# dellytools/delly

Hardware: AMD Instinct MI355X
Metric: candidate split-read alignments/sec (DEL, 150bp reads, 1kb ref window) (higher is better)
Workload: dtype int32-exact (uint8 / int16 storage)

## Files before the change

### delly_amd/csrc/sparse_needle.hpp

```cpp
#pragma once
#include <type_traits>

#ifndef DH_SP_CALLS
#define DH_SP_FN __forceinline__
#else
#define DH_SP_FN __noinline__
#endif

#include "split_kernel.hpp"

namespace dh {

constexpr int SP_NEG = -30000;
constexpr int SP_INF = 0x3fffffff;
constexpr int SP_LEVELS_MAX = 512;
constexpr int SP_UNKNOWN = -(1 << 30);

struct SparseWs {
  int16_t* frF;
  int16_t* frR;
  int32_t* cF;
  int32_t* cR;
  int32_t* runsF;
  int32_t* runsR;
  int32_t* listF;
  int32_t* listR;
  int32_t ndp;
  int32_t smax;
  int32_t pred_cap;
  int32_t runs_cap;
};

struct SparseRes {
  int resolved;
  int found;
  int unsplit;
  int best, consLeft, refLeft, refRight;
  int nrunsF, nrunsR;
  int levels;
  int mmF, mmR;
  unsigned long long t[5];
  int runF, runR;
};

typedef const __attribute__((address_space(1))) uint32_t* sp_gu32;
__device__ __forceinline__ int sp_ld16(const int16_t* p) {
  const uintptr_t u = reinterpret_cast<uintptr_t>(p);
  const uint32_t v = __hip_atomic_load((sp_gu32)(u & ~(uintptr_t)3), __ATOMIC_RELAXED, __HIP_MEMORY_SCOPE_AGENT);
  return (int)(int16_t)((u & 2) ? (v >> 16) : (v & 0xffffu));
}
__device__ __forceinline__ int sp_ld32(const int32_t* p) {
  return (int)__hip_atomic_load((sp_gu32) reinterpret_cast<uintptr_t>(p), __ATOMIC_RELAXED, __HIP_MEMORY_SCOPE_AGENT);
}

__device__ __forceinline__ int sp_ld8(const uint8_t* p) {
  const uintptr_t u = reinterpret_cast<uintptr_t>(p);
  const uint32_t v = __hip_atomic_load((sp_gu32)(u & ~(uintptr_t)3), __ATOMIC_RELAXED, __HIP_MEMORY_SCOPE_AGENT);
  return (int)((v >> (8 * (u & 3))) & 0xffu);
}

struct FrGlobal16 {
  const int16_t* base;
  int ndp;
  __device__ __forceinline__ int get(int d, int q) const { return sp_ld16(base + (size_t)d * ndp + q); }
};
struct FrTile8 {
  const uint8_t* base;
  int ndp;
  const uint8_t* row0;
  const uint8_t* row1;
  int S;
  __device__ __forceinline__ int get(int d, int q) const {
    return (d >= S - 1) ? (int)((d & 1) ? row1 : row0)[q] - 1 : sp_ld8(base + (size_t)d * ndp + q) - 1;
  }
};

__device__ __forceinline__ uint64_t sp_load8(const uint8_t* p) {
  uint64_t v;
  __builtin_memcpy(&v, p, 8);
  return v;
}

__device__ __forceinline__ uint64_t sp_lds8u(const uint8_t* p) {
  uint64_t v;
  __builtin_memcpy(&v, p, 8);
  return v;
}

constexpr int SP_LB = 16;
template <int TW, int STRCAP, typename ELEM = int16_t, int NROWS = 3>
struct __attribute__((aligned(16))) SpTileT {
  typedef ELEM elem_t;
  static constexpr int tw = TW;
  static constexpr int row_len = TW + 2 * SP_LB + 64;
  static constexpr int str_cap = STRCAP;
  static constexpr bool narrow = sizeof(ELEM) == 1;
  ELEM row[2][NROWS][TW + 2 * SP_LB + 64];
  uint8_t str[STRCAP > 0 ? STRCAP : 8];
};
typedef SpTileT<960, 8192, int16_t, 2> SpTile;

template <typename TILE, bool STAGED>
__device__ __forceinline__ void sp_tile_levels(const uint8_t* aF, const uint8_t* bF, const uint8_t* aR, const uint8_t* bR, int c0, int m, int n,
                                               int d0, int nl, int tlo, int thi, int16_t* FRf, int16_t* FRr, int ndp, TILE& T,
                                               int16_t* reachF, int16_t* reachR, int lane) {
  constexpr int OFF = SP_LB + 1;
  const int ND = n + m + 1;
  const int base = tlo - OFF;
  auto ld8 = [&](const uint8_t* p) -> uint64_t { return STAGED ? sp_lds8a(p) : sp_load8(p); };
  for (int j = 0; j < nl; ++j) {
    const int d = d0 + j;
    const int halo = nl - 1 - j;
    const int qa = max(tlo - halo, 0), qb = min(thi + halo, ND);
    int16_t* curF = T.row[0][d & 1] - base;
    int16_t* curR = T.row[1][d & 1] - base;
    const int16_t* p1F = T.row[0][(d + 1) & 1] - base;
    const int16_t* p1R = T.row[1][(d + 1) & 1] - base;
    const int16_t* p2F = curF;
    const int16_t* p2R = curR;
    int16_t* gF = FRf + (size_t)d * ndp;
    int16_t* gR = FRr + (size_t)d * ndp;
    const int seed = (d == 0) ? 0 : -1;
    int rf = -1, rr = -1;
    for (int q0 = qa; q0 < qb; q0 += 2 * WAVE) {
      int bf[2], br[2], kk[2];
      uint64_t zf[2], zr[2];
#pragma unroll
      for (int u = 0; u < 2; ++u) {
        const int q = min(q0 + u * WAVE + lane, qb - 1);
        const int k = q - m;
        kk[u] = k;
        const int nk = n - k, rmax = min(m, nk);
        const int first = (k < 0 && -2 * k <= d) ? -k : ((k >= 0) ? seed : -1);
        bf[u] = br[u] = first;
        if (d > 0) {
          {
            const int v1 = p1F[q], v1l = p1F[q - 1], v2 = p2F[q], v2r = p2F[q + 1];
            int b = max(v1, first);
            if ((unsigned)v1l <= (unsigned)nk) b = max(b, v1l);
            if (v2 >= 0) b = max(b, min(v2 + 1, rmax));
            if (v2r >= 0 && v2r < m) b = max(b, v2r + 1);
            bf[u] = b;
          }
          {
            const int v1 = p1R[q], v1l = p1R[q - 1], v2 = p2R[q], v2r = p2R[q + 1];
            int b = max(v1, first);
            if ((unsigned)v1l <= (unsigned)nk) b = max(b, v1l);
            if (v2 >= 0) b = max(b, min(v2 + 1, rmax));
            if (v2r >= 0 && v2r < m) b = max(b, v2r + 1);
            br[u] = b;
          }
        }
        const int r0 = max(bf[u], 0), r1 = max(br[u], 0);
        zf[u] = ld8(aF + r0) ^ ld8(bF + (max(r0 + k, c0) - c0));
        zr[u] = ld8(aR + r1) ^ ld8(bR + (max(r1 + k, c0) - c0));
      }
      int endF[2], endR[2];
      bool moreF[2], moreR[2];
#pragma unroll
      for (int u = 0; u < 2; ++u) {
        const int k = kk[u];
        {
          const int b0 = max(bf[u], 0);
          const int lim = min(m - b0, n - b0 - k);
          const int adv = zf[u] ? (int)(__builtin_ctzll(zf[u]) >> 3) : 8;
          endF[u] = b0 + lim;
          moreF[u] = bf[u] >= 0 && adv >= 8 && lim > 8;
          bf[u] = (bf[u] < 0) ? -1 : b0 + min(adv, lim);
        }
        {
          const int b0 = max(br[u], 0);
          const int lim = min(m - b0, n - b0 - k);
          const int adv = zr[u] ? (int)(__builtin_ctzll(zr[u]) >> 3) : 8;
          endR[u] = b0 + lim;
          moreR[u] = br[u] >= 0 && adv >= 8 && lim > 8;
          br[u] = (br[u] < 0) ? -1 : b0 + min(adv, lim);
        }
      }
#pragma unroll
      for (int u = 0; u < 2; ++u) {
        const int q = q0 + u * WAVE + lane, k = kk[u];
        if (__ballot(moreF[u])) {
          if (moreF[u]) {
            int r = bf[u];
            for (;;) {
              const uint64_t z = ld8(aF + r) ^ ld8(bF + (r + k - c0));
              if (z) { r += (int)(__builtin_ctzll(z) >> 3); break; }
              r += 8;
              if (r >= endF[u]) break;
            }
            bf[u] = min(r, endF[u]);
          }
        }
        if (__ballot(moreR[u])) {
          if (moreR[u]) {
            int r = br[u];
            for (;;) {
              const uint64_t z = ld8(aR + r) ^ ld8(bR + (r + k - c0));
              if (z) { r += (int)(__builtin_ctzll(z) >> 3); break; }
              r += 8;
              if (r >= endR[u]) break;
            }
            br[u] = min(r, endR[u]);
          }
        }
        if (q < qb) {
          curF[q] = (int16_t)bf[u];
          curR[q] = (int16_t)br[u];
          if (q >= tlo && q < thi) {
            gF[q] = (int16_t)bf[u];
            gR[q] = (int16_t)br[u];
            rf = max(rf, bf[u]);
            rr = max(rr, br[u]);
          }
        }
      }
    }
#pragma unroll
    for (int o = 32; o >= 1; o >>= 1) {
      rf = max(rf, __shfl_xor(rf, o));
      rr = max(rr, __shfl_xor(rr, o));
    }
    if (lane == 0) {
      reachF[d] = (int16_t)max((int)reachF[d], rf < 0 ? SP_NEG : rf);
      reachR[d] = (int16_t)max((int)reachR[d], rr < 0 ? SP_NEG : rr);
    }
// ... 47 lines not shown
}

#ifdef DH_SPS_DBG
__device__ unsigned long long dh_dbg[16];
#define DH_DBG_ADD(i, v) do { if (lane == 0) atomicAdd(&dh_dbg[i], (unsigned long long)(v)); } while (0)
#define DH_DBG_T() wall_clock64()
#else
#define DH_DBG_ADD(i, v) do { } while (0)
#define DH_DBG_T() 0ull
#endif
#ifdef DH_SPS_FINE
__shared__ unsigned long long dh_tl[6];
#define DH_TL(i) do { if (lane == 0) dh_tl[i] = wall_clock64(); } while (0)
#else
#define DH_TL(i) do { } while (0)
#endif
constexpr int SPS_OFF = 20;

template <bool NEG, bool EDGE>
__device__ __forceinline__ uint32_t sps_entries4(const uint8_t* cons, const uint8_t* ref, uint32_t e1, uint32_t e1l, uint32_t e2, uint32_t e2r,
                                                 int qb, int m, int n, int dhalf, int seed1, int ND, int& maxB, uint32_t& pend, int pbit) {
  int Bv[4], r0v[4], rmaxv[4];
  uint64_t zv[4];
#pragma unroll
  for (int i = 0; i < 4; ++i) {
    const int q = qb + i, k = q - m;
    const int E1 = (int)((e1 >> (8 * i)) & 255u), E1L = (int)((e1l >> (8 * i)) & 255u);
    const int E2 = (int)((e2 >> (8 * i)) & 255u), E2R = (int)((e2r >> (8 * i)) & 255u);
    int rmax = m;
    int B = E1;
    if (EDGE) {
      const int nk = n - k;
      rmax = min(m, nk);
      if ((unsigned)(E1L - 1) <= (unsigned)nk) B = max(B, E1L);
    } else {
      B = max(B, E1L);
    }
    B = max(B, E2 ? min(E2 + 1, rmax + 1) : 0);
    B = max(B, ((unsigned)(E2R - 1) < (unsigned)m) ? E2R + 1 : 0);
    if (NEG) {
      const int kk = -k;
      if ((unsigned)(kk - 1) < (unsigned)dhalf) B = max(B, kk + 1);
      B = max(B, (k >= 0) ? seed1 : 0);
    } else {
      B = max(B, seed1);
    }
    Bv[i] = B;
    rmaxv[i] = rmax;
    r0v[i] = max(B - 1, 0);
  }
#pragma unroll
  for (int i = 0; i < 4; ++i) {
    const int k = qb + i - m;
    zv[i] = sp_lds8a(cons + r0v[i]) ^ sp_lds8a(ref + (NEG ? max(r0v[i] + k, 0) : r0v[i] + k));
  }
  uint32_t outw = 0;
#pragma unroll
  for (int i = 0; i < 4; ++i) {
    const int q = qb + i;
    const int adv = zv[i] ? (int)(__builtin_ctzll(zv[i]) >> 3) : 8;
    int NB = Bv[i] ? min(r0v[i] + adv, rmaxv[i]) + 1 : 0;
    bool more = (Bv[i] != 0) && (adv >= 8) && (rmaxv[i] - r0v[i] > 8);
    if (EDGE) {
      NB = (q < ND) ? NB : 0;
      more = more && (q < ND);
    }
    outw |= (uint32_t)NB << (8 * i);
    maxB = max(maxB, NB);
    pend |= (more ? 1u : 0u) << (pbit + i);
  }
  return outw;
}

__device__ __forceinline__ void sps_extend_pending(const uint8_t* consF, const uint8_t* refF, const uint8_t* consR, const uint8_t* refR,
                                                   uint8_t* curF, uint8_t* curR, int q0, int m, int n, uint32_t pend, int& maxB_F,
                                                   int& maxB_R, int lane) {
  int total = 0;
#pragma unroll
  for (int e = 0; e < 8; ++e) total += __popcll(__ballot((pend >> e) & 1u));
  if (total > 6) {
#pragma unroll
    for (int e = 0; e < 8; ++e) {
      const bool mine = (pend >> e) & 1u;
      if (__ballot(mine) == 0ull) continue;
      if (mine) {
        const bool rev = e >= 4;
        const int q = q0 + 4 * lane + (e & 3), k = q - m;
        const uint8_t* cons = rev ? consR : consF;
        const uint8_t* ref = rev ? refR : refF;
        uint8_t* cur = rev ? curR : curF;
        const int end = min(m, n - k);
        int r = (int)cur[q] - 1;
        for (;;) {
          const uint64_t z = sp_lds8a(cons + r) ^ sp_lds8a(ref + r + k);
          if (z) { r += (int)(__builtin_ctzll(z) >> 3); break; }
          r += 8;
          if (r >= end) break;
        }
        r = min(r, end);
        cur[q] = (uint8_t)(r + 1);
        if (rev) maxB_R = max(maxB_R, r + 1); else maxB_F = max(maxB_F, r + 1);
      }
    }
    return;
  }
  unsigned long long lanes = __ballot(pend != 0u);
  while (lanes) {
    const int src = __builtin_ctzll(lanes);
    lanes &= lanes - 1;
    uint32_t bits = (uint32_t)__builtin_amdgcn_readlane((int)pend, src);
    while (bits) {
      const int e = __builtin_ctz(bits);
      bits &= bits - 1;
      const bool rev = e >= 4;
      const int q = q0 + 4 * src + (e & 3), k = q - m;
      const uint8_t* cons = rev ? consR : consF;
      const uint8_t* ref = rev ? refR : refF;
      uint8_t* cur = rev ? curR : curF;
      const int end = min(m, n - k);
      int r = (int)cur[q] - 1;
      for (;;) {
        const int rr = r + 8 * lane;
        uint64_t z = 0;
        if (rr < end) z = sp_lds8a(cons + rr) ^ sp_lds8a(ref + rr + k);
        const unsigned long long stop = __ballot(rr >= end || z != 0ull);
        if (stop == 0ull) { r += 8 * WAVE; continue; }
        const int jl = __builtin_ctzll(stop);
        const int rj = r + 8 * jl;
        const uint32_t zlo = (uint32_t)__builtin_amdgcn_readlane((int)(uint32_t)(z & 0xffffffffull), jl);
        const uint32_t zhi = (uint32_t)__builtin_amdgcn_readlane((int)(uint32_t)(z >> 32), jl);
        const uint64_t zz = ((uint64_t)zhi << 32) | zlo;
        r = (rj >= end) ? end : min(rj + (zz ? (int)(__builtin_ctzll(zz) >> 3) : 8), end);
        break;
      }
      if (lane == 0) cur[q] = (uint8_t)(r + 1);
      if (rev) maxB_R = max(maxB_R, r + 1); else maxB_F = max(maxB_F, r + 1);
    }
  }
}

template <bool NEG, bool EDGE, bool L0>
__device__ __forceinline__ uint32_t sps_level_step(const uint8_t* consF, const uint8_t* refF, const uint8_t* consR, const uint8_t* refR, int m, int n,
                                               int d, int q0, int ND, uint8_t* curF, uint8_t* curR, const uint8_t* p1F, const uint8_t* p1R,
                                               uint8_t* gF, uint8_t* gR, int& maxB_F, int& maxB_R, int lane) {
  const int qb = q0 + 4 * lane;
  uint32_t e1F = 0, e1lF = 0, e2F = 0, e2rF = 0, e1R = 0, e1lR = 0, e2R = 0, e2rR = 0;
  if (!L0) {
    const uint32_t* a1F = reinterpret_cast<const uint32_t*>(p1F + qb);
    const uint32_t* a2F = reinterpret_cast<const uint32_t*>(curF + qb);
    const uint32_t* a1R = reinterpret_cast<const uint32_t*>(p1R + qb);
    const uint32_t* a2R = reinterpret_cast<const uint32_t*>(curR + qb);
    e1F = a1F[0]; e1lF = __builtin_amdgcn_alignbyte(e1F, a1F[-1], 3u); e2F = a2F[0]; e2rF = __builtin_amdgcn_alignbyte(a2F[1], e2F, 1u);
    e1R = a1R[0]; e1lR = __builtin_amdgcn_alignbyte(e1R, a1R[-1], 3u); e2R = a2R[0]; e2rR = __builtin_amdgcn_alignbyte(a2R[1], e2R, 1u);
    if (d >= 2 && qb < ND) {
      *reinterpret_cast<uint32_t*>(gF + qb) = e2F;
      *reinterpret_cast<uint32_t*>(gR + qb) = e2R;
    }
  }
  uint32_t pend = 0;
  const int seed1 = L0 ? 1 : 0, dhalf = d >> 1;
  const uint32_t oF = sps_entries4<NEG, EDGE>(consF, refF, e1F, e1lF, e2F, e2rF, qb, m, n, dhalf, seed1, ND, maxB_F, pend, 0);
  __builtin_amdgcn_sched_barrier(0);
  const uint32_t oR = sps_entries4<NEG, EDGE>(consR, refR, e1R, e1lR, e2R, e2rR, qb, m, n, dhalf, seed1, ND, maxB_R, pend, 4);
  if (qb < ND) {
    *reinterpret_cast<uint32_t*>(curF + qb) = oF;
    *reinterpret_cast<uint32_t*>(curR + qb) = oR;
  }
  return pend;
}

template <typename TILE>
__device__ DH_SP_FN void sps_level_block(const uint8_t* consF, const uint8_t* refF, const uint8_t* consR, const uint8_t* refR, int m,
                                         int n, int d0, int d1, int16_t* FRf, int16_t* FRr, int ndp, TILE& T, int16_t* reachF,
                                         int16_t* reachR, int lane) {
  static_assert(TILE::narrow, "byte rows");
  static_assert(sizeof(T.row[0][0]) % 4 == 0 && SPS_OFF % 4 == 0, "dword access to the tile rows");
  const int ND = n + m + 1;
  const unsigned long long tz0 = DH_DBG_T();
  DH_TL(0);
  if (d0 == 0) {
    static_assert(sizeof(T.row) % 16 == 0 && alignof(TILE) >= 16, "the tile is cleared sixteen bytes per lane and store");
    uint4* z = reinterpret_cast<uint4*>(&T.row[0][0][0]);
    for (int i = lane; i < (int)(sizeof(T.row) / 16); i += WAVE) z[i] = make_uint4(0u, 0u, 0u, 0u);
  }
  __syncthreads();
  DH_TL(1);
  DH_DBG_ADD(0, 1);
  DH_DBG_ADD(7, DH_DBG_T() - tz0);
  for (int d = d0; d <= d1; ++d) {
    const unsigned long long tl0 = DH_DBG_T();
    uint8_t* curF = T.row[0][d & 1] + SPS_OFF;
    uint8_t* curR = T.row[1][d & 1] + SPS_OFF;
    const uint8_t* p1F = T.row[0][(d + 1) & 1] + SPS_OFF;
    const uint8_t* p1R = T.row[1][(d + 1) & 1] + SPS_OFF;
    uint8_t* gF = reinterpret_cast<uint8_t*>(FRf) + (size_t)max(d - 2, 0) * ndp;
    uint8_t* gR = reinterpret_cast<uint8_t*>(FRr) + (size_t)max(d - 2, 0) * ndp;
    int maxB_F = 0, maxB_R = 0;
    for (int q0 = 0; q0 < ND; q0 += 4 * WAVE) {
      const bool neg = q0 < m;
      const bool edge = q0 + 4 * WAVE - 1 > n;
      uint32_t pend;
      if (d == 0) {
        if (neg || edge) pend = sps_level_step<true, true, true>(consF, refF, consR, refR, m, n, d, q0, ND, curF, curR, p1F, p1R, gF, gR, maxB_F, maxB_R, lane);
        else pend = sps_level_step<false, false, true>(consF, refF, consR, refR, m, n, d, q0, ND, curF, curR, p1F, p1R, gF, gR, maxB_F, maxB_R, lane);
      } else if (neg || edge) {
        pend = sps_level_step<true, true, false>(consF, refF, consR, refR, m, n, d, q0, ND, curF, curR, p1F, p1R, gF, gR, maxB_F, maxB_R, lane);
      } else {
        pend = sps_level_step<false, false, false>(consF, refF, consR, refR, m, n, d, q0, ND, curF, curR, p1F, p1R, gF, gR, maxB_F, maxB_R, lane);
      }
      if (__ballot(pend != 0u)) {
        const unsigned long long te = DH_DBG_T();
        sps_extend_pending(consF, refF, consR, refR, curF, curR, q0, m, n, pend, maxB_F, maxB_R, lane);
        DH_DBG_ADD(5, 1);
        DH_DBG_ADD(6, DH_DBG_T() - te);
      }
    }
    const unsigned long long tl1 = DH_DBG_T();
    DH_TL(2);
#pragma unroll
    for (int o = 32; o >= 1; o >>= 1) {
      maxB_F = max(maxB_F, __shfl_xor(maxB_F, o));
      maxB_R = max(maxB_R, __shfl_xor(maxB_R, o));
    }
    if (lane == 0) {
      reachF[d] = (int16_t)(maxB_F <= 0 ? SP_NEG : maxB_F - 1);
      reachR[d] = (int16_t)(maxB_R <= 0 ? SP_NEG : maxB_R - 1);
    }
    __syncthreads();
    DH_DBG_ADD(1, 1);
    DH_DBG_ADD(2, tl1 - tl0);
    DH_DBG_ADD(3, DH_DBG_T() - tl1);
  }
  const unsigned long long tw0 = DH_DBG_T();
  if (d1 >= 2) asm volatile("s_waitcnt vmcnt(0)" ::: "memory");
  __syncthreads();
  DH_TL(3);
  DH_DBG_ADD(4, DH_DBG_T() - tw0);
}

template <typename TILE>
__device__ DH_SP_FN void sps_level_block_v1(const uint8_t* consF, const uint8_t* refF, const uint8_t* consR, const uint8_t* refR, int m,
                                             int n, int d0, int d1, int16_t* FRf, int16_t* FRr, int ndp, TILE& T, int16_t* reachF,
                                             int16_t* reachR, int lane) {
  static_assert(TILE::narrow, "byte rows");
  constexpr int OFF = SPS_OFF;
  const int ND = n + m + 1;
  if (d0 == 0) {
    uint32_t* z = reinterpret_cast<uint32_t*>(&T.row[0][0][0]);
    for (int i = lane; i < (int)(sizeof(T.row) / 4); i += WAVE) z[i] = 0u;
  }
  __syncthreads();
  for (int d = d0; d <= d1; ++d) {
    uint8_t* curF = T.row[0][d & 1] + OFF;
    uint8_t* curR = T.row[1][d & 1] + OFF;
    const uint8_t* p1F = T.row[0][(d + 1) & 1] + OFF;
    const uint8_t* p2F = curF;
    const uint8_t* p1R = T.row[1][(d + 1) & 1] + OFF;
    const uint8_t* p2R = curR;
    uint8_t* gF = reinterpret_cast<uint8_t*>(FRf) + (size_t)max(d - 2, 0) * ndp;
    uint8_t* gR = reinterpret_cast<uint8_t*>(FRr) + (size_t)max(d - 2, 0) * ndp;
    const int seed = (d == 0) ? 0 : -1;
    int rf = -1, rr = -1;
    for (int q0 = 0; q0 < ND; q0 += 2 * WAVE) {
      int bf[2], br[2], kk[2];
      uint64_t zf[2], zr[2];
#pragma unroll
      for (int u = 0; u < 2; ++u) {
        const int q = min(q0 + u * WAVE + lane, ND - 1);
        const int k = q - m;
        kk[u] = k;
        const int nk = n - k, rmax = min(m, nk);
        const int first = (k < 0 && -2 * k <= d) ? -k : ((k >= 0) ? seed : -1);
        bf[u] = br[u] = first;
        if (d > 0) {
          if (d >= 2 && q0 + u * WAVE + lane < ND) {
            gF[q] = p2F[q];
            gR[q] = p2R[q];
          }
          {
            const int e1 = p1F[q], e1l = p1F[q - 1], e2 = p2F[q], e2r = p2F[q + 1];
            int b = max(e1 - 1, first);
            if ((unsigned)(e1l - 1) <= (unsigned)nk) b = max(b, e1l - 1);
            if (e2 >= 1) b = max(b, min(e2, rmax));
            if (e2r >= 1 && e2r <= m) b = max(b, e2r);
            bf[u] = b;
          }
          {
            const int e1 = p1R[q], e1l = p1R[q - 1], e2 = p2R[q], e2r = p2R[q + 1];
            int b = max(e1 - 1, first);
            if ((unsigned)(e1l - 1) <= (unsigned)nk) b = max(b, e1l - 1);
            if (e2 >= 1) b = max(b, min(e2, rmax));
            if (e2r >= 1 && e2r <= m) b = max(b, e2r);
            br[u] = b;
          }
        }
        const int r0 = max(bf[u], 0), r1 = max(br[u], 0);
        zf[u] = sp_lds8u(consF + r0) ^ sp_lds8u(refF + max(r0 + k, 0));
        zr[u] = sp_lds8u(consR + r1) ^ sp_lds8u(refR + max(r1 + k, 0));
      }
      int endF[2], endR[2];
      bool moreF[2], moreR[2];
#pragma unroll
      for (int u = 0; u < 2; ++u) {
        const int k = kk[u];
        {
          const int b0 = max(bf[u], 0);
          const int lim = min(m - b0, n - b0 - k);
          const int adv = zf[u] ? (int)(__builtin_ctzll(zf[u]) >> 3) : 8;
          endF[u] = b0 + lim;
          moreF[u] = bf[u] >= 0 && adv >= 8 && lim > 8;
          bf[u] = (bf[u] < 0) ? -1 : b0 + min(adv, lim);
        }
        {
          const int b0 = max(br[u], 0);
          const int lim = min(m - b0, n - b0 - k);
          const int adv = zr[u] ? (int)(__builtin_ctzll(zr[u]) >> 3) : 8;
          endR[u] = b0 + lim;
          moreR[u] = br[u] >= 0 && adv >= 8 && lim > 8;
          br[u] = (br[u] < 0) ? -1 : b0 + min(adv, lim);
        }
      }
#pragma unroll
      for (int u = 0; u < 2; ++u) {
        const int q = q0 + u * WAVE + lane, k = kk[u];
        if (__ballot(moreF[u])) {
          if (moreF[u]) {
            int r = bf[u];
            for (;;) {
              const uint64_t z = sp_lds8u(consF + r) ^ sp_lds8u(refF + r + k);
              if (z) { r += (int)(__builtin_ctzll(z) >> 3); break; }
              r += 8;
              if (r >= endF[u]) break;
            }
            bf[u] = min(r, endF[u]);
          }
        }
        if (__ballot(moreR[u])) {
          if (moreR[u]) {
            int r = br[u];
            for (;;) {
              const uint64_t z = sp_lds8u(consR + r) ^ sp_lds8u(refR + r + k);
              if (z) { r += (int)(__builtin_ctzll(z) >> 3); break; }
              r += 8;
              if (r >= endR[u]) break;
            }
            br[u] = min(r, endR[u]);
          }
        }
        if (q < ND) {
          curF[q] = (uint8_t)(bf[u] + 1);
          curR[q] = (uint8_t)(br[u] + 1);
          rf = max(rf, bf[u]);
          rr = max(rr, br[u]);
        }
      }
    }
#pragma unroll
    for (int o = 32; o >= 1; o >>= 1) {
      rf = max(rf, __shfl_xor(rf, o));
      rr = max(rr, __shfl_xor(rr, o));
    }
    if (lane == 0) {
      reachF[d] = (int16_t)(rf < 0 ? SP_NEG : rf);
      reachR[d] = (int16_t)(rr < 0 ? SP_NEG : rr);
    }
    __syncthreads();
  }
  asm volatile("s_waitcnt vmcnt(0)" ::: "memory");
  __syncthreads();
}

__device__ __forceinline__ void sp_offer_chunk(int32_t* row, int rlo, int rhi, int k, int v, int& pm, int lane) {
  if (__ballot(v > pm && v >= rlo) == 0ull) return;
  int incl = v;
#pragma unroll
  for (int o = 1; o < WAVE; o <<= 1) {
    const int t = __shfl_up(incl, o);
    if (lane >= o) incl = max(incl, t);
  }
  int excl = __shfl_up(incl, 1);
  if (lane == 0) excl = SP_NEG;
  const int from = max(max(excl, pm) + 1, rlo), to = min(v, rhi);
  const int hs = min(to, from + 7);
  for (int r = from; r <= hs; ++r) atomicMin(&row[r], r + k);
  unsigned long long todo = __ballot(to > from + 7);
  while (todo) {
    const int src = __builtin_ctzll(todo);
    todo &= todo - 1;
    const int f2 = __shfl(from, src) + 8, t2 = __shfl(to, src), k2 = __shfl(k, src);
    for (int r = f2 + lane; r <= t2; r += WAVE) atomicMin(&row[r], r + k2);
  }
  pm = max(pm, __shfl(incl, WAVE - 1));
}
template <typename FRV>
__device__ __forceinline__ void sp_offer_negative(const FRV& FR, int32_t* row, int m, int d, int rlo, int rhi, int lane) {
  const int nneg = min(d / 2, m);
  for (int i0 = 0; i0 < nneg; i0 += WAVE) {
    const int i = i0 + lane;
    const int v = (i < nneg) ? FR.get(d, m - 1 - i) : SP_NEG;
    const int cnt = min(WAVE, nneg - i0);
    for (int t = 0; t < cnt; ++t) {
      const int vt = __shfl(v, t), kt = -(i0 + t + 1);
      const int lo = max(rlo, -kt), hi = min(vt, rhi);
      for (int r = lo + lane; r <= hi; r += WAVE) atomicMin(&row[r], r + kt);
    }
  }
}

template <typename FRV>
__device__ DH_SP_FN void sp_first_columns(const FRV& FR, int m, int n, int S, int rlo, int rhi, int32_t* cT, int lane) {
  const int ND = n + m + 1;
  const int rows = rhi - rlo + 1;
  for (int d = 0; d <= S; ++d)
    for (int i = lane; i < rows; i += WAVE) cT[(size_t)d * (m + 1) + rlo + i] = SP_INF;
  asm volatile("s_waitcnt vmcnt(0)" ::: "memory");
  __syncthreads();
  for (int d0 = 0; d0 <= S; d0 += 4) {
    int pm[4];
#pragma unroll
    for (int u = 0; u < 4; ++u) {
      pm[u] = (d0 + u <= S) ? rlo - 1 : rhi;
      if (d0 + u <= S) sp_offer_negative(FR, cT + (size_t)(d0 + u) * (m + 1), m, d0 + u, rlo, rhi, lane);
    }
    for (int q0 = m; q0 < ND && (pm[0] < rhi || pm[1] < rhi || pm[2] < rhi || pm[3] < rhi); q0 += WAVE) {
      const int q = q0 + lane;
      int v[4];
#pragma unroll
      for (int u = 0; u < 4; ++u) v[u] = (q < ND && pm[u] < rhi) ? FR.get(min(d0 + u, S), q) : SP_NEG;
#pragma unroll
      for (int u = 0; u < 4; ++u)
        if (pm[u] < rhi) sp_offer_chunk(cT + (size_t)(d0 + u) * (m + 1), rlo, rhi, q - m, v[u], pm[u], lane);
    }
  }
  asm volatile("s_waitcnt vmcnt(0)" ::: "memory");
  __syncthreads();
}

template <typename FRV>
__device__ DH_SP_FN int sp_deep_list(const FRV& FR, int m, int n, int S, int rlo, int32_t* list, int cap, int lane) {
  const int ND = n + m + 1;
  int cnt = 0;
  for (int q0 = 0; q0 < ND; q0 += WAVE) {
    const int q = q0 + lane;
    const bool hit = (q < ND) && (FR.get(S, min(q, ND - 1)) >= rlo);
    const unsigned long long bm = __ballot(hit);
    if (bm) {
      const unsigned long long below = (lane == 0) ? 0ull : (~0ull >> (64 - lane));
      const int pos = cnt + __popcll(bm & below);
      if (hit && pos < cap) list[pos] = q;
      cnt += __popcll(bm);
    }
  }
  asm volatile("s_waitcnt vmcnt(0)" ::: "memory");
  __syncthreads();
  return (cnt <= cap) ? cnt : -1;
}

template <bool WAIT = true>
__device__ __forceinline__ int sps_deep_list(const uint8_t* lv, int ND, int rlo, int32_t* list, int cap, int lane) {
  int cnt = 0;
  for (int q0 = 0; q0 < ND; q0 += WAVE) {
    const int q = q0 + lane;
    const bool hit = (q < ND) && ((int)lv[min(q, ND - 1)] - 1 >= rlo);
    const unsigned long long bm = __ballot(hit);
    if (bm) {
      const unsigned long long below = (lane == 0) ? 0ull : (~0ull >> (64 - lane));
      const int pos = cnt + __popcll(bm & below);
      if (hit && pos < cap) list[pos] = q;
      cnt += __popcll(bm);
    }
  }
  if (WAIT) {
    asm volatile("s_waitcnt vmcnt(0)" ::: "memory");
    __syncthreads();
  }
  return (cnt <= cap) ? cnt : -1;
}

template <typename FRV>
__device__ DH_SP_FN void sp_first_columns_list(const FRV& FR, int m, int S, int rlo, int rhi, const int32_t* list,
                                                   int cnt, int32_t* cT, int lane) {
  const int rows = rhi - rlo + 1;
  for (int d = 0; d <= S; ++d)
    for (int i = lane; i < rows; i += WAVE) cT[(size_t)d * (m + 1) + rlo + i] = SP_INF;
  asm volatile("s_waitcnt vmcnt(0)" ::: "memory");
  __syncthreads();
  if (cnt <= WAVE) {
    const int q = (lane < cnt) ? sp_ld32(list + lane) : -1;
    const bool use = q >= m;
    for (int d0 = 0; d0 <= S; d0 += 4) {
      int v[4];
#pragma unroll
      for (int u = 0; u < 4; ++u) v[u] = (use && d0 + u <= S) ? FR.get(d0 + u, q) : SP_NEG;
#pragma unroll
      for (int u = 0; u < 4; ++u) {
        if (d0 + u <= S) {
          int pm = rlo - 1;
          sp_offer_chunk(cT + (size_t)(d0 + u) * (m + 1), rlo, rhi, q - m, v[u], pm, lane);
        }
      }
    }
  } else {
    for (int d = 0; d <= S; ++d) {
      int pm = rlo - 1;
      for (int i0 = 0; i0 < cnt && pm < rhi; i0 += WAVE) {
        const int i = i0 + lane;
        const int q = (i < cnt) ? sp_ld32(list + i) : -1;
        const int v = (q >= m) ? FR.get(d, q) : SP_NEG;
        sp_offer_chunk(cT + (size_t)d * (m + 1), rlo, rhi, q - m, v, pm, lane);
      }
    }
  }
  for (int d = 2; d <= S; ++d) sp_offer_negative(FR, cT + (size_t)d * (m + 1), m, d, rlo, rhi, lane);
  asm volatile("s_waitcnt vmcnt(0)" ::: "memory");
  __syncthreads();
}

template <typename FRV>
__device__ DH_SP_FN void sp_first_columns_both(const FRV& FRf, const FRV& FRr, int m, int S, int rloF, int rhiF,
                                                   const int32_t* listF, int cntF, int32_t* cF, int rloR, int rhiR,
                                                   const int32_t* listR, int cntR, int32_t* cR, int lane) {
  const int rows = rhiF - rloF + 1;
  for (int d = 0; d <= S; ++d)
    for (int i = lane; i < rows; i += WAVE) {
      cF[(size_t)d * (m + 1) + rloF + i] = SP_INF;
      cR[(size_t)d * (m + 1) + rloR + i] = SP_INF;
    }
  asm volatile("s_waitcnt vmcnt(0)" ::: "memory");
  __syncthreads();
  const int qF = (lane < cntF) ? sp_ld32(listF + lane) : -1;
  const int qR = (lane < cntR) ? sp_ld32(listR + lane) : -1;
  const bool useF = qF >= m, useR = qR >= m;
  for (int d0 = 0; d0 <= S; d0 += 4) {
    int vF[4], vR[4];
#pragma unroll
    for (int u = 0; u < 4; ++u) {
      vF[u] = (useF && d0 + u <= S) ? FRf.get(d0 + u, qF) : SP_NEG;
      vR[u] = (useR && d0 + u <= S) ? FRr.get(d0 + u, qR) : SP_NEG;
    }
#pragma unroll
    for (int u = 0; u < 4; ++u) {
      if (d0 + u <= S) {
        int pmF = rloF - 1, pmR = rloR - 1;
        sp_offer_chunk(cF + (size_t)(d0 + u) * (m + 1), rloF, rhiF, qF - m, vF[u], pmF, lane);
        sp_offer_chunk(cR + (size_t)(d0 + u) * (m + 1), rloR, rhiR, qR - m, vR[u], pmR, lane);
      }
    }
  }
  for (int d = 2; d <= S; ++d) {
    sp_offer_negative(FRf, cF + (size_t)d * (m + 1), m, d, rloF, rhiF, lane);
    sp_offer_negative(FRr, cR + (size_t)d * (m + 1), m, d, rloR, rhiR, lane);
  }
  asm volatile("s_waitcnt vmcnt(0)" ::: "memory");
  __syncthreads();
}

template <typename FRV, bool REGRUNS = false>
__device__ DH_SP_FN int sp_trace(const FRV& FR, int m, int n, int r, int c, int D, int32_t* runs, int cap, int lane,
                                     int* mismatches = nullptr, int* runreg = nullptr) {
  const int ND = n + m + 1;
  const int D0 = rfl(D);
  int nv = 0, nh = 0;
  auto fr = [&](int d, int q) -> int { return (d < 0 || q < 0 || q >= ND) ? SP_NEG : FR.get(d, q); };
  int nruns = 0, last_op = -1, last_len = 0;
  auto emit = [&](int op, int len) {
    if (len <= 0) return;
    if (op == last_op) { last_len += len; return; }
    if (last_op >= 0) {
      if (REGRUNS) { if (lane == nruns) *runreg = (last_op << 24) | last_len; }
      else if (nruns < cap && lane == 0) runs[nruns] = (last_op << 24) | last_len;
      ++nruns;
    }
    last_op = op;
    last_len = len;
  };
  r = rfl(r); c = rfl(c); D = rfl(D);
  while (r > 0 || c > 0) {
    if (r == 0) { emit(2, c); c = 0; break; }
    if (c == 0) { emit(1, r); nv += r; r = 0; break; }
    const int k = c - r, q = k + m;
    if (D >= 2 && rfl(fr(D - 2, q + 1)) >= r - 1) { emit(1, 1); ++nv; --r; D -= 2; continue; }
    if (D >= 1 && rfl(fr(D - 1, q - 1)) >= r) { emit(2, 1); ++nh; --c; D -= 1; continue; }
    const int lowD = (D >= 1) ? max(rfl(fr(D - 1, q)) + 1, 0) : 0;
    int T = SP_NEG;
    if (D >= 2) T = max(T, rfl(fr(D - 2, q + 1)) + 1);
    if (D >= 1) T = max(T, rfl(fr(D - 1, q - 1)));
    const int start = max(0, -k);
    const int y = max(max(lowD, T + 1), start + 1);
    const int cnt = r - y + 1;
    emit(0, cnt);
    r -= cnt;
    c -= cnt;
    if (r < lowD) {
      int e = D - 1;
      while (e >= 1 && rfl(fr(e - 1, q)) >= r) --e;
      D = (rfl(fr(e, q)) >= r) ? e : D;
    }
  }
  if (last_op >= 0) {
    if (REGRUNS) { if (lane == nruns) *runreg = (last_op << 24) | last_len; }
    else if (nruns < cap && lane == 0) runs[nruns] = (last_op << 24) | last_len;
    ++nruns;
  }
  if (mismatches) *mismatches = (D0 - 2 * nv - nh) / 2;
  if (!REGRUNS) {
    asm volatile("s_waitcnt vmcnt(0)" ::: "memory");
    __syncthreads();
  }
  return (nruns <= (REGRUNS ? WAVE : cap)) ? nruns : -1;
}

struct SpsSmall {
  int qF, qR, nF, nR;
  uint32_t pF[3], pR[3];
};

template <typename FRV>
__device__ __forceinline__ bool sps_lists_small(const FRV& frF, const FRV& frR, const uint8_t* lvF, const uint8_t* lvR, int ND, int m, int SE,
                                                int rlo, int rloR, SpsSmall& Q, int lane) {
  Q.qF = Q.qR = -1;
  int nF = 0, nR = 0;
  for (int q0 = 0; q0 < ND; q0 += 4 * WAVE) {
    const int qb = q0 + 4 * lane;
    const uint32_t wf = *reinterpret_cast<const uint32_t*>(lvF + qb), wr = *reinterpret_cast<const uint32_t*>(lvR + qb);
    uint32_t hf = 0u, hr = 0u;
#pragma unroll
    for (int i = 0; i < 4; ++i) {
      const bool in = qb + i < ND;
      hf |= (uint32_t)(in && (int)((wf >> (8 * i)) & 255u) - 1 >= rlo) << i;
      hr |= (uint32_t)(in && (int)((wr >> (8 * i)) & 255u) - 1 >= rloR) << i;
    }
    if (__ballot((hf | hr) != 0u) == 0ull) continue;
#pragma unroll
    for (int i = 0; i < 4; ++i) {
      unsigned long long bf = __ballot((hf >> i) & 1u), br = __ballot((hr >> i) & 1u);
      if (nF + __popcll(bf) > WAVE || nR + __popcll(br) > WAVE) return false;
      while (bf) {
        const int b = __builtin_ctzll(bf);
        bf &= bf - 1;
        Q.qF = (lane == nF) ? q0 + 4 * b + i : Q.qF;
        ++nF;
      }
      while (br) {
        const int b = __builtin_ctzll(br);
        br &= br - 1;
        Q.qR = (lane == nR) ? q0 + 4 * b + i : Q.qR;
        ++nR;
      }
    }
  }
  Q.nF = nF;
  Q.nR = nR;
#pragma unroll
  for (int w = 0; w < 3; ++w) { Q.pF[w] = 0u; Q.pR[w] = 0u; }
#pragma unroll
  for (int d = 0; d < 9; ++d) {
    if (d <= SE) {
      const int vf = (Q.qF >= 0) ? frF.get(d, Q.qF) + 1 : 0;
      const int vr = (Q.qR >= 0) ? frR.get(d, Q.qR) + 1 : 0;
      Q.pF[d >> 2] |= (uint32_t)(vf & 255) << (8 * (d & 3));
      Q.pR[d >> 2] |= (uint32_t)(vr & 255) << (8 * (d & 3));
    }
  }
  return true;
}

template <int NL>
__device__ __forceinline__ void sps_row_best(const int (&lo_)[9], const int (&c2_)[9], int SE, int n, int r, long long& kb, int& db) {
  int thr[NL];
#pragma unroll
  for (int q = 0; q < NL; ++q) thr[q] = (q <= SE) ? ((c2_[q] > n) ? -1 : n - c2_[q]) : SP_INF;
#pragma unroll
  for (int d = 0; d < NL; ++d) {
    const int lo = lo_[d];
    int e = 0;
#pragma unroll
    for (int q = 0; q < NL; ++q) e += (int)(lo > thr[q]);
    const long long kk = ((long long)(d + e) << 40) | ((long long)r << 20) | (long long)lo;
    const bool take = (bool)((int)(d <= SE) & (int)(lo <= n) & (int)(e <= SE) & (int)(d + e <= SE) & (int)(kk <= kb));
    kb = take ? kk : kb;
    db = take ? d : db;
  }
}

template <int NL>
__device__ __forceinline__ void sps_join_small_t(const SpsSmall& Q, int m, int n, int SE, int rlo, int rhi, long long& key, int& dsel, int lane) {
  key = 0x7fffffffffffffffll;
  int dbest = 0;
  for (int r0 = rlo; r0 <= rhi; r0 += WAVE) {
    const int r = r0 + lane, rr = m - r;
    int lo_[9], c2_[9];
#pragma unroll
    for (int d = 0; d < 9; ++d) { lo_[d] = SP_INF; c2_[d] = SP_INF; }
    for (int t = 0; t < Q.nF; ++t) {
      const int k = __builtin_amdgcn_readlane(Q.qF, t) - m;
      const uint32_t p0 = (uint32_t)__builtin_amdgcn_readlane((int)Q.pF[0], t), p1 = (uint32_t)__builtin_amdgcn_readlane((int)Q.pF[1], t),
                     p2 = (uint32_t)__builtin_amdgcn_readlane((int)Q.pF[2], t);
      const bool on = r + k >= 0;
#pragma unroll
      for (int d = 0; d < NL; ++d) {
        if (d <= SE) {
          const int v = (int)((((d < 4) ? p0 : (d < 8) ? p1 : p2) >> (8 * (d & 3))) & 255u) - 1;
          lo_[d] = min(lo_[d], ((int)on & (int)(v >= r)) ? r + k : SP_INF);
        }
      }
    }
    for (int t = 0; t < Q.nR; ++t) {
      const int k = __builtin_amdgcn_readlane(Q.qR, t) - m;
      const uint32_t p0 = (uint32_t)__builtin_amdgcn_readlane((int)Q.pR[0], t), p1 = (uint32_t)__builtin_amdgcn_readlane((int)Q.pR[1], t),
                     p2 = (uint32_t)__builtin_amdgcn_readlane((int)Q.pR[2], t);
      const bool on = rr + k >= 0;
#pragma unroll
      for (int d = 0; d < NL; ++d) {
        if (d <= SE) {
          const int v = (int)((((d < 4) ? p0 : (d < 8) ? p1 : p2) >> (8 * (d & 3))) & 255u) - 1;
          c2_[d] = min(c2_[d], ((int)on & (int)(v >= rr)) ? rr + k : SP_INF);
        }
      }
    }
    if (r <= rhi) {
      long long kb = 0x7fffffffffffffffll;
      int db = 0;
      sps_row_best<NL>(lo_, c2_, SE, n, r, kb, db);
      if (kb < key) { key = kb; dbest = db; }
    }
  }
  long long kmin = key;
#pragma unroll
  for (int o = 32; o >= 1; o >>= 1) {
    const int lo = __shfl_xor((int)(kmin & 0xffffffffll), o), hi = __shfl_xor((int)(kmin >> 32), o);
    const long long w = ((long long)hi << 32) | (unsigned int)lo;
    kmin = w < kmin ? w : kmin;
  }
  const unsigned long long who = __ballot(key == kmin && key != 0x7fffffffffffffffll);
  dsel = who ? __shfl(dbest, __builtin_ctzll(who)) : 0;
  key = kmin;
}
__device__ __forceinline__ void sps_join_small(const SpsSmall& Q, int m, int n, int SE, int rlo, int rhi, long long& key, int& dsel, int lane) {
  if (SE <= 0) sps_join_small_t<1>(Q, m, n, SE, rlo, rhi, key, dsel, lane);
  else if (SE <= 2) sps_join_small_t<3>(Q, m, n, SE, rlo, rhi, key, dsel, lane);
  else sps_join_small_t<9>(Q, m, n, SE, rlo, rhi, key, dsel, lane);
}

template <typename TILE, bool LDSSTR>
__device__ DH_SP_FN SparseRes sparse_long_needle(const uint8_t* cons, const uint8_t* rcons, const uint8_t* ref, const uint8_t* rref,
                                                    int m, int n, const SparseWs& W, TILE& T, int16_t* reachF, int16_t* reachR,
                                                    int s_first, int lane) {
  SparseRes O;
  O.resolved = 0; O.found = 0; O.unsplit = SP_UNKNOWN; O.best = 0; O.consLeft = O.refLeft = O.refRight = 0; O.nrunsF = O.nrunsR = 0; O.levels = 0; O.mmF = O.mmR = 0;
  const int ND = n + m + 1;
  if (ND + 1 > W.ndp || m < 1 || n < 1 || W.smax < 4) return O;
  int done = -1;
  int S = min(W.smax, s_first);
  for (;;) {
    if constexpr (LDSSTR && TILE::narrow) {
#ifdef DH_SPS_LEVEL_V1
      sps_level_block_v1(cons, ref, rcons, rref, m, n, done + 1, S, W.frF, W.frR, W.ndp, T, reachF, reachR, lane);
#else
      sps_level_block(cons, ref, rcons, rref, m, n, done + 1, S, W.frF, W.frR, W.ndp, T, reachF, reachR, lane);
#endif
    } else {
      for (int d = done + 1; d <= S; d += SP_LB)
        sp_level_block2<TILE>(cons, ref, rcons, rref, m, n, d, min(d + SP_LB - 1, S), W.frF, W.frR, W.ndp, T, reachF, reachR, lane);
    }
    __syncthreads();
#ifdef DH_LR_TIMING
    O.t[0] = wall_clock64();
#endif
    done = S;
    constexpr bool TILED8 = LDSSTR && TILE::narrow;
    typedef typename std::conditional<TILED8, FrTile8, FrGlobal16>::type FRV;
    FRV frF, frR;
    if constexpr (TILED8) {
      frF = FrTile8{reinterpret_cast<const uint8_t*>(W.frF), W.ndp, &T.row[0][0][0] + SPS_OFF, &T.row[0][1][0] + SPS_OFF, S};
      frR = FrTile8{reinterpret_cast<const uint8_t*>(W.frR), W.ndp, &T.row[1][0][0] + SPS_OFF, &T.row[1][1][0] + SPS_OFF, S};
    } else {
      frF = FrGlobal16{W.frF, W.ndp};
      frR = FrGlobal16{W.frR, W.ndp};
    }
    int du = -1;
    for (int d0 = 0; d0 <= S && du < 0; d0 += WAVE) {
      const int d = d0 + lane;
      const unsigned long long hit = __ballot(d <= S && reachF[d] >= m);
      if (hit) du = d0 + __builtin_ctzll(hit);
    }
    const int SE = (du >= 0) ? min(S, du - 1) : S;
    const int rhi = (SE >= 0) ? min(m, (int)reachF[max(SE, 0)]) : -1, rlo = (SE >= 0) ? max(0, m - (int)reachR[max(SE, 0)]) : 0;
    long long key = 0x7fffffffffffffffll;
    int dsel = 0;
    int nlistR = -1;
    bool feasible = false;
    for (int d0 = 0; SE >= 0 && d0 <= SE && !feasible; d0 += WAVE) {
      const int d = d0 + lane;
      feasible = __ballot(d <= SE && reachF[min(d, SE)] >= 0 && (int)reachR[SE - min(d, SE)] >= m - (int)reachF[min(d, SE)]) != 0ull;
    }
    bool small = false;
    SpsSmall Q;
    if constexpr (LDSSTR && TILE::narrow) {
      if (rlo <= rhi && feasible && SE >= S - 1 && SE <= 8) {
        small = sps_lists_small(frF, frR, T.row[0][SE & 1] + SPS_OFF, T.row[1][SE & 1] + SPS_OFF, ND, m, SE, rlo, m - rhi, Q, lane);
        if (small) {
#ifdef DH_LR_TIMING
          O.t[1] = wall_clock64();
#endif
          sps_join_small(Q, m, n, SE, rlo, rhi, key, dsel, lane);
        }
      }
    }
    if (rlo <= rhi && feasible && !small) {
      int nlistF;
      bool tables_done = false;
      if constexpr (LDSSTR && TILE::narrow) {
        if (SE >= S - 1) {
          nlistF = sps_deep_list<false>(T.row[0][SE & 1] + SPS_OFF, ND, rlo, W.listF, W.runs_cap, lane);
          nlistR = sps_deep_list<false>(T.row[1][SE & 1] + SPS_OFF, ND, m - rhi, W.listR, W.runs_cap, lane);
        } else {
          nlistF = sp_deep_list(frF, m, n, SE, rlo, W.listF, W.runs_cap, lane);
          nlistR = sp_deep_list(frR, m, n, SE, m - rhi, W.listR, W.runs_cap, lane);
        }
        if (nlistF >= 0 && nlistF <= WAVE && nlistR >= 0 && nlistR <= WAVE) {
          sp_first_columns_both(frF, frR, m, SE, rlo, rhi, W.listF, nlistF, W.cF, m - rhi, m - rlo, W.listR, nlistR, W.cR, lane);
          tables_done = true;
        } else {
          asm volatile("s_waitcnt vmcnt(0)" ::: "memory");
          __syncthreads();
        }
      } else {
        nlistF = sp_deep_list(frF, m, n, SE, rlo, W.listF, W.runs_cap, lane);
        nlistR = sp_deep_list(frR, m, n, SE, m - rhi, W.listR, W.runs_cap, lane);
      }
      if (!tables_done) {
        if (nlistF >= 0) sp_first_columns_list(frF, m, SE, rlo, rhi, W.listF, nlistF, W.cF, lane);
        else sp_first_columns(frF, m, n, SE, rlo, rhi, W.cF, lane);
        if (nlistR >= 0) sp_first_columns_list(frR, m, SE, m - rhi, m - rlo, W.listR, nlistR, W.cR, lane);
        else sp_first_columns(frR, m, n, SE, m - rhi, m - rlo, W.cR, lane);
      }
#ifdef DH_LR_TIMING
      O.t[1] = wall_clock64();
#endif
      int dbest = 0;
      for (int r0 = rlo; r0 <= rhi; r0 += WAVE) {
        const int r = r0 + lane;
        if (r <= rhi) {
          long long kb = 0x7fffffffffffffffll;
          int db = 0;
          const int32_t* cf = W.cF + r;
          const int32_t* cr = W.cR + (m - r);
          if (SE <= 8) {
            int lo_[9], c2_[9];
#pragma unroll
            for (int q = 0; q < 9; ++q) {
              lo_[q] = (q <= SE) ? sp_ld32(cf + (size_t)q * (m + 1)) : SP_INF;
              c2_[q] = (q <= SE) ? sp_ld32(cr + (size_t)q * (m + 1)) : SP_INF;
            }
            sps_row_best<9>(lo_, c2_, SE, n, r, kb, db);
          } else {
          int e = SE + 1;
          for (int d = 0; d <= SE; ++d) {
            const int lo = sp_ld32(cf + (size_t)d * (m + 1));
            if (lo > n) continue;
            while (e >= 1) {
              const int c2 = sp_ld32(cr + (size_t)(e - 1) * (m + 1));
              if (c2 <= n && lo <= n - c2) --e;
              else break;
            }
            if (e <= SE && d + e <= SE) {
              const long long kk = ((long long)(d + e) << 40) | ((long long)r << 20) | (long long)lo;
              if (kk <= kb) { kb = kk; db = d; }
            }
          }
          }
          if (kb < key) { key = kb; dbest = db; }
        }
      }
      long long kmin = key;
#pragma unroll
      for (int o = 32; o >= 1; o >>= 1) {
        const int lo = __shfl_xor((int)(kmin & 0xffffffffll), o), hi = __shfl_xor((int)(kmin >> 32), o);
        const long long w = ((long long)hi << 32) | (unsigned int)lo;
        kmin = w < kmin ? w : kmin;
      }
      const unsigned long long who = __ballot(key == kmin && key != 0x7fffffffffffffffll);
      dsel = who ? __shfl(dbest, __builtin_ctzll(who)) : 0;
      key = kmin;
    }
#ifdef DH_LR_TIMING
    O.t[2] = wall_clock64();
#endif
    const bool have = key != 0x7fffffffffffffffll;
    const int bestD = have ? (int)(key >> 40) : -1;
    if (du >= 0 || have) {
      O.resolved = 1;
      O.levels = S;
      O.unsplit = (du >= 0) ? m - du : SP_UNKNOWN;
      if (!have || (du >= 0 && bestD >= du)) {
        O.found = 0;
        O.best = m - du;
        return O;
      }
      O.found = 1;
      O.best = m - bestD;
      O.consLeft = (int)((key >> 20) & 0xfffff);
      O.refLeft = (int)(key & 0xfffff);
      const int cr_ = m - O.consLeft;
      const int eR = bestD - dsel;
      int rright = 0;
      if (small) {
        const int w = eR >> 2, sh = 8 * (eR & 3);
        const uint32_t pw = (w == 0) ? Q.pR[0] : (w == 1) ? Q.pR[1] : Q.pR[2];
        const int v = (int)((pw >> sh) & 255u) - 1;
        const int t = cr_ + Q.qR - m;
        if (Q.qR >= 0 && t >= 0 && t <= n - O.refLeft && v >= cr_) rright = t;
      } else if (nlistR >= 0) {
        for (int i0 = 0; i0 < nlistR; i0 += WAVE) {
          const int i = i0 + lane;
          if (i < nlistR) {
            const int q = sp_ld32(W.listR + i), k = q - m, t = cr_ + k;
            if (t >= 0 && t <= n - O.refLeft && frR.get(eR, q) >= cr_) rright = max(rright, t);
          }
        }
      } else {
        for (int q0 = 0; q0 < ND; q0 += WAVE) {
          const int q = q0 + lane;
          if (q < ND) {
            const int k = q - m, t = cr_ + k;
            if (t >= 0 && t <= n - O.refLeft && frR.get(eR, q) >= cr_) rright = max(rright, t);
          }
        }
      }
#pragma unroll
      for (int o = 32; o >= 1; o >>= 1) rright = max(rright, __shfl_xor(rright, o));
      O.refRight = rfl(rright);
#ifdef DH_LR_TIMING
      O.t[3] = wall_clock64();
#endif
      if constexpr (LDSSTR && TILE::narrow) {
        O.runF = O.runR = 0;
        O.nrunsF = sp_trace<FRV, true>(frF, m, n, O.consLeft, O.refLeft, dsel, W.runsF, W.runs_cap, lane, &O.mmF, &O.runF);
        O.nrunsR = sp_trace<FRV, true>(frR, m, n, cr_, O.refRight, eR, W.runsR, W.runs_cap, lane, &O.mmR, &O.runR);
      } else {
        O.nrunsF = sp_trace(frF, m, n, O.consLeft, O.refLeft, dsel, W.runsF, W.runs_cap, lane, &O.mmF);
        O.nrunsR = sp_trace(frR, m, n, cr_, O.refRight, eR, W.runsR, W.runs_cap, lane, &O.mmR);
      }
#ifdef DH_LR_TIMING
      O.t[4] = wall_clock64();
#endif
      if (O.nrunsF < 0 || O.nrunsR < 0) O.resolved = 0;
      return O;
    }
    if (S >= W.smax) return O;
    {
      const long long covered = max(1, (int)reachF[S] + (int)reachR[S]);
      const long long pred = (2ll * S * m) / covered;
      if (pred > W.pred_cap) return O;
    }
    S = min(W.smax, (S < (LDSSTR ? 16 : 8)) ? S + 2 : (S < 32) ? S * 2 : S + SP_LB);
  }
}

struct RunsMem {
  const int32_t* p;
  __device__ __forceinline__ int at(int i) const { return rfl(sp_ld32(p + i)); }
  __device__ __forceinline__ int mine(int i, int n) const { return (i >= 0 && i < n) ? sp_ld32(p + i) : 0; }
};
struct RunsReg {
  int r;
  __device__ __forceinline__ int at(int i) const { return __builtin_amdgcn_readlane(r, i); }
  __device__ __forceinline__ int mine(int i, int n) const { const int v = __shfl(r, max(min(i, WAVE - 1), 0)); return (i >= 0 && i < n) ? v : 0; }
};

template <typename PL, typename APPEND, typename RUNS = RunsMem>
__device__ __forceinline__ int sparse_masks_t(PL& L, RUNS runsF, int nF, RUNS runsR, int nR, int gapref, int maskw,
                                              int lane, int& posC, APPEND append) {
  for (int w = lane; w < maskw; w += WAVE) {
    L.mV[w] = 0;
    L.mR[w] = 0;
    L.mE[w] = 0;
  }
  __syncthreads();
  int pos = 0;
  auto put = [&](int op, int len) {
    const unsigned long long v = (op != 2) ? ~0ull : 0ull, r = (op != 1) ? ~0ull : 0ull;
    for (int k = 0; k < len; k += 64) {
      append(L, pos, min(64, len - k), v, r, lane);
      pos += min(64, len - k);
    }
  };
  for (int i = nF - 1; i >= 0; --i) {
    const int x = runsF.at(i);
    put(x >> 24, x & 0xffffff);
  }
  put(2, gapref);
  posC = pos;
  for (int i = 0; i < nR; ++i) {
    const int x = runsR.at(i);
    put(x >> 24, x & 0xffffff);
  }
  return pos;
}

// ... 112 lines not shown
```

Before: 64.77 million.

## Recompute level-0 frontier on demand and skip its global spill

Level 0 of the byte frontier is no longer written to global memory. FrTile8::get recomputes it by comparing consensus and reference 8 bytes at a time, and the store and vmcnt wait now start from level 3 instead of 2. The cF/cR pointers are also derived from the frR workspace base and pinned in scalar registers, and an asm barrier on lane is added to steer codegen. This saves global stores and waits in the level loop. In exchange, any later read of level 0 pays the recompute cost, and the change relies on the derived workspace layout matching W.cF and W.cR.

```diff
diff --git a/delly_amd/csrc/sparse_needle.hpp b/delly_amd/csrc/sparse_needle.hpp
--- a/delly_amd/csrc/sparse_needle.hpp
+++ b/delly_amd/csrc/sparse_needle.hpp
@@ -70,8 +70,25 @@
   const uint8_t* row0;
   const uint8_t* row1;
   int S;
+  const uint8_t* cons;
+  const uint8_t* ref;
+  int m, n;
+  __device__ __forceinline__ int level0(int q) const {
+    const int k = q - m;
+    if (k < 0 || k > n) return -1;
+    const int end = min(m, n - k);
+    int r = 0;
+    while (r < end) {
+      const uint64_t z = sp_lds8a(cons + r) ^ sp_lds8a(ref + r + k);
+      if (z) { r += (int)(__builtin_ctzll(z) >> 3); break; }
+      r += 8;
+    }
+    return min(r, end);
+  }
   __device__ __forceinline__ int get(int d, int q) const {
-    return (d >= S - 1) ? (int)((d & 1) ? row1 : row0)[q] - 1 : sp_ld8(base + (size_t)d * ndp + q) - 1;
+    if (d >= S - 1) return (int)((d & 1) ? row1 : row0)[q] - 1;
+    if (d == 0) return level0(q);
+    return sp_ld8(base + (size_t)d * ndp + q) - 1;
   }
 };
 
@@ -425,7 +442,7 @@
     const uint32_t* a2R = reinterpret_cast<const uint32_t*>(curR + qb);
     e1F = a1F[0]; e1lF = __builtin_amdgcn_alignbyte(e1F, a1F[-1], 3u); e2F = a2F[0]; e2rF = __builtin_amdgcn_alignbyte(a2F[1], e2F, 1u);
     e1R = a1R[0]; e1lR = __builtin_amdgcn_alignbyte(e1R, a1R[-1], 3u); e2R = a2R[0]; e2rR = __builtin_amdgcn_alignbyte(a2R[1], e2R, 1u);
-    if (d >= 2 && qb < ND) {
+    if (d >= 3 && qb < ND) {
       *reinterpret_cast<uint32_t*>(gF + qb) = e2F;
       *reinterpret_cast<uint32_t*>(gR + qb) = e2R;
     }
@@ -505,7 +522,7 @@
     DH_DBG_ADD(3, DH_DBG_T() - tl1);
   }
   const unsigned long long tw0 = DH_DBG_T();
-  if (d1 >= 2) asm volatile("s_waitcnt vmcnt(0)" ::: "memory");
+  if (d1 >= 3) asm volatile("s_waitcnt vmcnt(0)" ::: "memory");
   __syncthreads();
   DH_TL(3);
   DH_DBG_ADD(4, DH_DBG_T() - tw0);
@@ -793,6 +810,7 @@
 __device__ DH_SP_FN void sp_first_columns_both(const FRV& FRf, const FRV& FRr, int m, int S, int rloF, int rhiF,
                                                    const int32_t* listF, int cntF, int32_t* cF, int rloR, int rhiR,
                                                    const int32_t* listR, int cntR, int32_t* cR, int lane) {
+  asm volatile("" : "+v"(lane));
   const int rows = rhiF - rloF + 1;
   for (int d = 0; d <= S; ++d)
     for (int i = lane; i < rows; i += WAVE) {
@@ -1045,11 +1063,21 @@
     typedef typename std::conditional<TILED8, FrTile8, FrGlobal16>::type FRV;
     FRV frF, frR;
     if constexpr (TILED8) {
-      frF = FrTile8{reinterpret_cast<const uint8_t*>(W.frF), W.ndp, &T.row[0][0][0] + SPS_OFF, &T.row[0][1][0] + SPS_OFF, S};
-      frR = FrTile8{reinterpret_cast<const uint8_t*>(W.frR), W.ndp, &T.row[1][0][0] + SPS_OFF, &T.row[1][1][0] + SPS_OFF, S};
+      frF = FrTile8{reinterpret_cast<const uint8_t*>(W.frF), W.ndp, &T.row[0][0][0] + SPS_OFF, &T.row[0][1][0] + SPS_OFF, S, cons, ref, m, n};
+      frR = FrTile8{reinterpret_cast<const uint8_t*>(W.frR), W.ndp, &T.row[1][0][0] + SPS_OFF, &T.row[1][1][0] + SPS_OFF, S, rcons, rref, m, n};
     } else {
       frF = FrGlobal16{W.frF, W.ndp};
       frR = FrGlobal16{W.frR, W.ndp};
+    }
+    int32_t* cF = W.cF;
+    int32_t* cR = W.cR;
+    if constexpr (TILED8) {
+      const uintptr_t f = reinterpret_cast<uintptr_t>(W.frR) + (size_t)(W.smax + 1) * W.ndp;
+      const uintptr_t r = f + (size_t)(W.smax + 1) * (m + 1) * 4;
+      uint32_t flo = (uint32_t)f, fhi = (uint32_t)(f >> 32), rlo_ = (uint32_t)r, rhi_ = (uint32_t)(r >> 32);
+      asm volatile("" : "+s"(flo), "+s"(fhi), "+s"(rlo_), "+s"(rhi_));
+      cF = reinterpret_cast<int32_t*>(((uintptr_t)fhi << 32) | flo);
+      cR = reinterpret_cast<int32_t*>(((uintptr_t)rhi_ << 32) | rlo_);
     }
     int du = -1;
     for (int d0 = 0; d0 <= S && du < 0; d0 += WAVE) {
@@ -1092,7 +1120,7 @@
           nlistR = sp_deep_list(frR, m, n, SE, m - rhi, W.listR, W.runs_cap, lane);
         }
         if (nlistF >= 0 && nlistF <= WAVE && nlistR >= 0 && nlistR <= WAVE) {
-          sp_first_columns_both(frF, frR, m, SE, rlo, rhi, W.listF, nlistF, W.cF, m - rhi, m - rlo, W.listR, nlistR, W.cR, lane);
+          sp_first_columns_both(frF, frR, m, SE, rlo, rhi, W.listF, nlistF, cF, m - rhi, m - rlo, W.listR, nlistR, cR, lane);
           tables_done = true;
         } else {
           asm volatile("s_waitcnt vmcnt(0)" ::: "memory");
@@ -1103,10 +1131,10 @@
         nlistR = sp_deep_list(frR, m, n, SE, m - rhi, W.listR, W.runs_cap, lane);
       }
       if (!tables_done) {
-        if (nlistF >= 0) sp_first_columns_list(frF, m, SE, rlo, rhi, W.listF, nlistF, W.cF, lane);
-        else sp_first_columns(frF, m, n, SE, rlo, rhi, W.cF, lane);
-        if (nlistR >= 0) sp_first_columns_list(frR, m, SE, m - rhi, m - rlo, W.listR, nlistR, W.cR, lane);
-        else sp_first_columns(frR, m, n, SE, m - rhi, m - rlo, W.cR, lane);
+        if (nlistF >= 0) sp_first_columns_list(frF, m, SE, rlo, rhi, W.listF, nlistF, cF, lane);
+        else sp_first_columns(frF, m, n, SE, rlo, rhi, cF, lane);
+        if (nlistR >= 0) sp_first_columns_list(frR, m, SE, m - rhi, m - rlo, W.listR, nlistR, cR, lane);
+        else sp_first_columns(frR, m, n, SE, m - rhi, m - rlo, cR, lane);
       }
 #ifdef DH_LR_TIMING
       O.t[1] = wall_clock64();
@@ -1117,8 +1145,8 @@
         if (r <= rhi) {
           long long kb = 0x7fffffffffffffffll;
           int db = 0;
-          const int32_t* cf = W.cF + r;
-          const int32_t* cr = W.cR + (m - r);
+          const int32_t* cf = cF + r;
+          const int32_t* cr = cR + (m - r);
           if (SE <= 8) {
             int lo_[9], c2_[9];
 #pragma unroll
```

After: 65.59 million (median of 6 runs). +1.3%, better.
